# SonyResearch/micro_diffusion

Measured on AMD Instinct MI355X. Metric: training images/sec (global batch 2048) MicroDiT-XL/2 256-res mask=0.75, higher is better.
Workload: dtype bf16; 1 GPU; MicroDiT_XL_2 res_256_pretrain.yaml mask=0.75, full step = 2 microbatches x 1024 fwd+bwd + grad exchange + clip 0.25 + AdamW; global_batch=2048, microbatch=1024, parallelism=dp1, grad_exchange=none (single rank)

## Files before the change

micro_diffusion_amd/csrc/attention.hip:

```cpp
#include <stdlib.h>
#include "md_common.h"
#include "../../include/microdit_hip.h"

namespace {

typedef __attribute__((address_space(3))) s16x4 lds_s16x4;
typedef unsigned int u32x4 __attribute__((ext_vector_type(4)));

__device__ __forceinline__ bf16x4 tr4(const unsigned char* p) {
    s16x4 v = __builtin_amdgcn_ds_read_tr16_b64_v4i16((lds_s16x4*)(p));
    U64 t;
    t.s = v;
    return t.h;
}

__device__ __forceinline__ bf16x8 tr_frag(const unsigned char* tile, int pitch, int k_lo, int k_hi, int col0, int lane) {
    const int li = lane & 15;
    const int col = col0 + ((lane >> 4) & 1) * 16 + (li & 3) * 4;
    const bf16x4 lo = tr4(tile + (k_lo + (li >> 2)) * pitch + col * 2);
    const bf16x4 hi = tr4(tile + (k_hi + (li >> 2)) * pitch + col * 2);
    bf16x8 f;
    f[0] = lo[0]; f[1] = lo[1]; f[2] = lo[2]; f[3] = lo[3];
    f[4] = hi[0]; f[5] = hi[1]; f[6] = hi[2]; f[7] = hi[3];
    return f;
}

__device__ __forceinline__ bf16x8 row_frag(const unsigned char* tile, int pitch, int kbase, int lane) {
    U128 t;
    t.u = *reinterpret_cast<const uint4*>(tile + (lane & 31) * pitch + (kbase + (lane >> 5) * 8) * 2);
    return t.h;
}

template <int HD>
__device__ __forceinline__ void stage_tile(unsigned char* tile, int pitch, const bf16* src, int64_t ld, int64_t row0,
                                           int64_t nrows, int nstage, int tid, int nthreads) {
    constexpr int CPR = HD / 8;
    for (int task = tid; task < nstage * CPR; task += nthreads) {
        const int r = task / CPR, c = task % CPR;
        uint4 v = make_uint4(0, 0, 0, 0);
        if (row0 + r < nrows) v = *reinterpret_cast<const uint4*>(src + (row0 + r) * ld + c * 8);
        *reinterpret_cast<uint4*>(tile + r * pitch + c * 16) = v;
    }
}

constexpr int STG = 32;

template <int HD, int MAXIT>
__device__ __forceinline__ void stage_pair(unsigned char* tileA, unsigned char* tileB, int pitch, const bf16* A, int64_t lda, const bf16* B,
                                           int64_t ldb, int64_t row0, int64_t nrows, int nstage, int tid, int nthreads) {
    constexpr int CPR = HD / 8;
    uint4 ra[MAXIT], rb[MAXIT];
#pragma unroll
    for (int it = 0; it < MAXIT; ++it) {
        const int task = tid + it * nthreads, r = task / CPR, c = task % CPR;
        ra[it] = rb[it] = make_uint4(0, 0, 0, 0);
        if (task < nstage * CPR && row0 + r < nrows) {
            ra[it] = *reinterpret_cast<const uint4*>(A + (row0 + r) * lda + c * 8);
            rb[it] = *reinterpret_cast<const uint4*>(B + (row0 + r) * ldb + c * 8);
        }
    }
#pragma unroll
    for (int it = 0; it < MAXIT; ++it) {
        const int task = tid + it * nthreads, r = task / CPR, c = task % CPR;
        if (task < nstage * CPR) {
            *reinterpret_cast<uint4*>(tileA + r * pitch + c * 16) = ra[it];
            *reinterpret_cast<uint4*>(tileB + r * pitch + c * 16) = rb[it];
        }
    }
}

constexpr float LOG2E = 1.4426950408889634f;
__device__ __forceinline__ int tile_slot(int r, int hh) { return (r & 3) + 8 * (r >> 2) + 4 * hh; }

__device__ __forceinline__ void ds_cols(f32x16& s, const f32x16& dp, float c1, float l2, float dlt, int rem, int hh) {
#pragma unroll
    for (int r = 0; r < 16; ++r) {
        const float pr = tile_slot(r, hh) < rem ? __builtin_amdgcn_exp2f(s[r] * c1 - l2) : 0.f;
        s[r] = pr * (dp[r] - dlt);
    }
}
template <bool WANT_P, bool WANT_DS>
__device__ __forceinline__ void p_ds_rows(f32x16& s, f32x16& dp, float c1, const float* tL2, const float* tDlt, int rem, int hh) {
#pragma unroll
    for (int r = 0; r < 16; ++r) {
        const int ql = tile_slot(r, hh);
        const float pr = ql < rem ? __builtin_amdgcn_exp2f(s[r] * c1 - tL2[ql]) : 0.f;
        if (WANT_DS) dp[r] = pr * (dp[r] - tDlt[ql]);
        if (WANT_P) s[r] = pr;
    }
}
constexpr float LSE_MASKED = 1e30f;
template <bool WANT_P, bool WANT_DS, bool VEC = true>
__device__ __forceinline__ void p_ds_rows_nomask(f32x16& s, f32x16& dp, float c1, const float* tL2, const float* tDlt, int hh) {
    if (!VEC) {
#pragma unroll
        for (int r = 0; r < 16; ++r) {
            const int ql = tile_slot(r, hh);
            const float pr = __builtin_amdgcn_exp2f(s[r] * c1 - tL2[ql]);
            if (WANT_DS) dp[r] = pr * (dp[r] - tDlt[ql]);
            if (WANT_P) s[r] = pr;
        }
        return;
    }
#pragma unroll
    for (int j = 0; j < 4; ++j) {
        const f32x4 l4 = *reinterpret_cast<const f32x4*>(tL2 + 8 * j + 4 * hh);
        f32x4 d4 = {0.f, 0.f, 0.f, 0.f};
        if (WANT_DS) d4 = *reinterpret_cast<const f32x4*>(tDlt + 8 * j + 4 * hh);
#pragma unroll
        for (int e = 0; e < 4; ++e) {
            const int r = 4 * j + e;
            const float pr = __builtin_amdgcn_exp2f(s[r] * c1 - l4[e]);
            if (WANT_DS) dp[r] = pr * (dp[r] - d4[e]);
            if (WANT_P) s[r] = pr;
        }
    }
}

__device__ __forceinline__ bf16x8 pack8(const f32x16& a, int base) {
    bf16x8 o;
#pragma unroll
    for (int e = 0; e < 8; ++e) o[e] = f2bf(a[base + e]);
    return o;
}

__device__ __forceinline__ void bh_of(int64_t lin, int64_t H, int64_t B, int64_t& b, int64_t& h) {
    const int64_t n8 = (B >> 3) * 8 * H;
    if (lin < n8) {
        const int64_t s = lin >> 3, x = lin & 7;
        lin = ((s / H) * 8 + x) * H + s % H;
    }
    b = lin / H;
    h = lin - b * H;
}

enum : unsigned {
    SF_FWD_WIDE = 1u, SF_FWD_LINES = 2u,
    SF_FWDS_WIDE = 4u,
    SF_FUSED_WIDE = 8u, SF_FUSED_LINES = 16u,
    SF_FUSED2_LINES = 32u,
    SF_SPLIT2_WIDE = 64u,
    SF_STREAM_WIDE = 128u, SF_STREAM_LINES = 256u,
// ... 19 lines not shown

template <int HD>
__device__ __forceinline__ void store_rows(bf16* dst_row, const f32x16 (&acc)[HD / 32], float mul, int lane, bool wide) {
    const int hh = lane >> 5;
    if (wide) {
#pragma unroll
        for (int di = 0; di < HD / 32; ++di)
#pragma unroll
            for (int g = 0; g < 4; g += 2) {
                unsigned a0 = cvt_pk_bf16(acc[di][4 * g] * mul, acc[di][4 * g + 1] * mul);
                unsigned a1 = cvt_pk_bf16(acc[di][4 * g + 2] * mul, acc[di][4 * g + 3] * mul);
                unsigned b0 = cvt_pk_bf16(acc[di][4 * g + 4] * mul, acc[di][4 * g + 5] * mul);
                unsigned b1 = cvt_pk_bf16(acc[di][4 * g + 6] * mul, acc[di][4 * g + 7] * mul);
                half_swap(a0, b0);
                half_swap(a1, b1);
                *reinterpret_cast<uint4*>(dst_row + di * 32 + 8 * g + 8 * hh) = make_uint4(a0, a1, b0, b1);
            }
        return;
    }
#pragma unroll
    for (int di = 0; di < HD / 32; ++di)
#pragma unroll
        for (int g = 0; g < 4; ++g) {
            bf16x4 o;
#pragma unroll
            for (int e = 0; e < 4; ++e) o[e] = f2bf(acc[di][4 * g + e] * mul);
            st_bf16x4(dst_row + di * 32 + 8 * g + 4 * hh, o);
        }
}

template <int HD>
__device__ __forceinline__ void store_lines(unsigned char* tile, int pitch, bf16* dst0, int64_t ld, int nvalid, const f32x16 (&acc)[HD / 32],
                                            float mul, int lane) {
    const int hh = lane >> 5;
#pragma unroll
    for (int di = 0; di < HD / 32; ++di)
#pragma unroll
        for (int g = 0; g < 4; ++g)
            *reinterpret_cast<uint2*>(tile + (lane & 31) * pitch + (di * 32 + 8 * g + 4 * hh) * 2) =
                make_uint2(cvt_pk_bf16(acc[di][4 * g] * mul, acc[di][4 * g + 1] * mul), cvt_pk_bf16(acc[di][4 * g + 2] * mul, acc[di][4 * g + 3] * mul));
    __builtin_amdgcn_fence(__ATOMIC_RELEASE, "wavefront");
    __builtin_amdgcn_wave_barrier();
    constexpr int CPR = HD / 8, RPI = 64 / CPR;
#pragma unroll
    for (int it = 0; it < 32 / RPI; ++it) {
        const int r = it * RPI + lane / CPR, c = lane % CPR;
        const uint4 v = *reinterpret_cast<const uint4*>(tile + r * pitch + c * 16);
        if (r < nvalid) *reinterpret_cast<uint4*>(dst0 + r * ld + c * 8) = v;
    }
    __builtin_amdgcn_fence(__ATOMIC_ACQUIRE, "wavefront");
    __builtin_amdgcn_wave_barrier();
}

template <int HD, int MAXIT>
__global__ __launch_bounds__(256) void attn_fwd_kernel(md_attn_args p) {
    constexpr int PK = (HD + 8) * 2;
    __shared__ __attribute__((aligned(16))) unsigned char smem[2 * STG * PK];
    const int tid = threadIdx.x, lane = tid & 63, wave = tid >> 6, nthreads = blockDim.x, nw = nthreads >> 6;
    const int hh = lane >> 5;
    const float c1 = p.scale * LOG2E;
    int64_t b = blockIdx.z, h = blockIdx.y;
    if (gridDim.x == 1) bh_of(blockIdx.y + (int64_t)gridDim.y * blockIdx.z, gridDim.y, gridDim.z, b, h);
    const int64_t q = ((int64_t)blockIdx.x * nw + wave) * 32 + (lane & 31);
    const bool qvalid = q < p.Sq;
    const bf16* Q = reinterpret_cast<const bf16*>(p.q) + b * p.sq + h * p.hsq;
    const bf16* K = reinterpret_cast<const bf16*>(p.k) + b * p.sk + h * p.hsk;
    const bf16* V = reinterpret_cast<const bf16*>(p.v) + b * p.sv + h * p.hsv;

    bf16x8 qf[HD / 16];
#pragma unroll
    for (int s = 0; s < HD / 16; ++s) {
        if (qvalid)
            qf[s] = ld_bf16x8(Q + q * p.ldq + s * 16 + hh * 8);
        else
#pragma unroll
            for (int e = 0; e < 8; ++e) qf[s][e] = f2bf(0.f);
    }
    f32x16 oacc[HD / 32];
#pragma unroll
    for (int di = 0; di < HD / 32; ++di)
#pragma unroll
        for (int r = 0; r < 16; ++r) oacc[di][r] = 0.f;
    float m = -1e30f, l = 0.f;

    for (int64_t kbase = 0; kbase < p.Skv; kbase += STG) {
        __syncthreads();
        const int nst = (int)((p.Skv - kbase >= STG) ? STG : ((p.Skv - kbase + 31) / 32) * 32);
        stage_pair<HD, MAXIT>(smem, smem + STG * PK, PK, K, p.ldk, V, p.ldv, kbase, p.Skv, nst, tid, nthreads);
        __syncthreads();
      for (int sub = 0; sub < STG / 32 && kbase + sub * 32 < p.Skv; ++sub) {
        const int64_t key0 = kbase + sub * 32;
        const unsigned char* sK = smem + sub * 32 * PK;
        const unsigned char* sV = smem + STG * PK + sub * 32 * PK;
        f32x16 sacc;
#pragma unroll
        for (int r = 0; r < 16; ++r) sacc[r] = 0.f;
#pragma unroll
        for (int s = 0; s < HD / 16; ++s)
            sacc = __builtin_amdgcn_mfma_f32_32x32x16_bf16(row_frag(sK, PK, s * 16, lane), qf[s], sacc, 0, 0, 0);
        const int rem = (int)(p.Skv - key0);
        float tmax = -1e30f;
#pragma unroll
        for (int r = 0; r < 16; ++r) {
            sacc[r] = tile_slot(r, hh) < rem ? sacc[r] * c1 : -1e30f;
            tmax = fmaxf(tmax, sacc[r]);
        }
        tmax = fmaxf(tmax, __shfl_xor(tmax, 32, 64));
        const float m_new = fmaxf(m, tmax);
        const float alpha = __builtin_amdgcn_exp2f(m - m_new);
        float psum = 0.f;
#pragma unroll
        for (int r = 0; r < 16; ++r) {
            const float pr = __builtin_amdgcn_exp2f(sacc[r] - m_new);
            sacc[r] = pr;
            psum += pr;
        }
        psum += __shfl_xor(psum, 32, 64);
        l = l * alpha + psum;
        m = m_new;
#pragma unroll
        for (int di = 0; di < HD / 32; ++di)
#pragma unroll
            for (int r = 0; r < 16; ++r) oacc[di][r] *= alpha;
#pragma unroll
        for (int sp = 0; sp < 2; ++sp) {
            const bf16x8 pf = pack8(sacc, 8 * sp);
#pragma unroll
            for (int di = 0; di < HD / 32; ++di)
                oacc[di] = __builtin_amdgcn_mfma_f32_32x32x16_bf16(
                    tr_frag(sV, PK, 16 * sp + 4 * hh, 16 * sp + 8 + 4 * hh, di * 32, lane), pf, oacc[di], 0, 0, 0);
        }
      }
    }
    constexpr bool PLAIN = HD == 64 && MAXIT == 1;
    const bool o16 = rows16(p.o, p.ldo, p.so, p.hso);
    if (sf(SF_FWD_LINES) && !PLAIN && nw <= 2 && o16) {
        __syncthreads();
        const int64_t q0 = ((int64_t)blockIdx.x * nw + wave) * 32;
        const int nvalid = p.Sq - q0 >= 32 ? 32 : (p.Sq > q0 ? (int)(p.Sq - q0) : 0);
        store_lines<HD>(smem + wave * 32 * PK, PK, reinterpret_cast<bf16*>(p.o) + b * p.so + h * p.hso + q0 * p.ldo, p.ldo, nvalid, oacc,
                        1.f / l, lane);
    } else if (qvalid) {
        bf16* O = reinterpret_cast<bf16*>(p.o) + b * p.so + h * p.hso + q * p.ldo;
        store_rows<HD>(O, oacc, 1.f / l, lane, sf(SF_FWD_WIDE) && !PLAIN && o16);
    }
    if (qvalid && lane < 32 && p.lse) reinterpret_cast<float*>(p.lse)[(b * p.H + h) * p.Sq + q] = (m + __log2f(l)) * 0.6931471805599453f;
}


template <int HD, int MAXIT>
struct ChunkRegs {
    u32x4 a[MAXIT], b[MAXIT];
};
template <int HD, int SCH, int MAXIT>
__device__ __forceinline__ void chunk_load(ChunkRegs<HD, MAXIT>& R, const bf16* A, int64_t lda, const bf16* B, int64_t ldb, int64_t row0,
                                           int64_t nrows, int tid, int nthreads) {
    constexpr int CPR = HD / 8;
    const u32x4 z4 = {0u, 0u, 0u, 0u};
#pragma unroll
    for (int it = 0; it < MAXIT; ++it) {
        const int task = tid + it * nthreads, r = task / CPR, c = task % CPR;
        const bool ok = task < SCH * CPR && row0 + r < nrows;
        R.a[it] = ok ? *reinterpret_cast<const u32x4*>(A + (row0 + r) * lda + c * 8) : z4;
        R.b[it] = ok ? *reinterpret_cast<const u32x4*>(B + (row0 + r) * ldb + c * 8) : z4;
    }
}
template <int HD, int SCH, int MAXIT>
__device__ __forceinline__ void chunk_store(const ChunkRegs<HD, MAXIT>& R, unsigned char* tileA, unsigned char* tileB, int pitch, int tid,
                                            int nthreads) {
    constexpr int CPR = HD / 8;
#pragma unroll
    for (int it = 0; it < MAXIT; ++it) {
        const int task = tid + it * nthreads, r = task / CPR, c = task % CPR;
        if (task < SCH * CPR) {
            *reinterpret_cast<u32x4*>(tileA + r * pitch + c * 16) = R.a[it];
            *reinterpret_cast<u32x4*>(tileB + r * pitch + c * 16) = R.b[it];
        }
    }
}

template <int HD, int SCH, int MAXIT>
__global__ __launch_bounds__(512) void attn_fwd_stream_kernel(md_attn_args p) {
    constexpr int PK = (HD + 8) * 2;
    __shared__ __attribute__((aligned(16))) unsigned char smem[2 * SCH * PK];
    unsigned char* sKc = smem;
    unsigned char* sVc = smem + SCH * PK;
    const int tid = threadIdx.x, lane = tid & 63, wave = tid >> 6, nthreads = blockDim.x, nw = nthreads >> 6;
    const int hh = lane >> 5;
    const float c1 = p.scale * LOG2E;
    const int64_t b = blockIdx.z, h = blockIdx.y;
    const int64_t q = ((int64_t)blockIdx.x * nw + wave) * 32 + (lane & 31);
    const bool qvalid = q < p.Sq;
    const bf16* Q = reinterpret_cast<const bf16*>(p.q) + b * p.sq + h * p.hsq;
    const bf16* K = reinterpret_cast<const bf16*>(p.k) + b * p.sk + h * p.hsk;
    const bf16* V = reinterpret_cast<const bf16*>(p.v) + b * p.sv + h * p.hsv;

    ChunkRegs<HD, MAXIT> R;
    chunk_load<HD, SCH, MAXIT>(R, K, p.ldk, V, p.ldv, 0, p.Skv, tid, nthreads);
    bf16x8 qf[HD / 16];
#pragma unroll
    for (int s = 0; s < HD / 16; ++s) {
        if (qvalid)
            qf[s] = ld_bf16x8(Q + q * p.ldq + s * 16 + hh * 8);
        else
#pragma unroll
            for (int e = 0; e < 8; ++e) qf[s][e] = f2bf(0.f);
    }
    f32x16 oacc[HD / 32];
#pragma unroll
    for (int di = 0; di < HD / 32; ++di)
#pragma unroll
        for (int r = 0; r < 16; ++r) oacc[di][r] = 0.f;
    float m = -1e30f, l = 0.f;

    for (int64_t kbase = 0; kbase < p.Skv; kbase += SCH) {
        __syncthreads();
        chunk_store<HD, SCH, MAXIT>(R, sKc, sVc, PK, tid, nthreads);
        __syncthreads();
        if (kbase + SCH < p.Skv) chunk_load<HD, SCH, MAXIT>(R, K, p.ldk, V, p.ldv, kbase + SCH, p.Skv, tid, nthreads);
        auto tile = [&](int sub, int rem) {
            const unsigned char* sK = sKc + sub * 32 * PK;
            const unsigned char* sV = sVc + sub * 32 * PK;
            f32x16 sacc;
#pragma unroll
            for (int r = 0; r < 16; ++r) sacc[r] = 0.f;
#pragma unroll
            for (int s = 0; s < HD / 16; ++s)
                sacc = __builtin_amdgcn_mfma_f32_32x32x16_bf16(row_frag(sK, PK, s * 16, lane), qf[s], sacc, 0, 0, 0);
            float tmax = -1e30f;
#pragma unroll
            for (int r = 0; r < 16; ++r) {
                sacc[r] = tile_slot(r, hh) < rem ? sacc[r] * c1 : -1e30f;
                tmax = fmaxf(tmax, sacc[r]);
            }
            tmax = fmaxf(tmax, __shfl_xor(tmax, 32, 64));
            const float m_new = fmaxf(m, tmax);
            const float alpha = __builtin_amdgcn_exp2f(m - m_new);
            float psum = 0.f;
#pragma unroll
            for (int r = 0; r < 16; ++r) {
                const float pr = __builtin_amdgcn_exp2f(sacc[r] - m_new);
                sacc[r] = pr;
                psum += pr;
            }
            psum += __shfl_xor(psum, 32, 64);
            l = l * alpha + psum;
            m = m_new;
#pragma unroll
            for (int di = 0; di < HD / 32; ++di)
#pragma unroll
                for (int r = 0; r < 16; ++r) oacc[di][r] *= alpha;
#pragma unroll
            for (int sp = 0; sp < 2; ++sp) {
                const bf16x8 pf = pack8(sacc, 8 * sp);
#pragma unroll
                for (int di = 0; di < HD / 32; ++di)
                    oacc[di] = __builtin_amdgcn_mfma_f32_32x32x16_bf16(
                        tr_frag(sV, PK, 16 * sp + 4 * hh, 16 * sp + 8 + 4 * hh, di * 32, lane), pf, oacc[di], 0, 0, 0);
            }
        };
        if (kbase + SCH <= p.Skv) {
#pragma unroll 1
            for (int sub = 0; sub < SCH / 32; ++sub) tile(sub, 32);
        } else {
            for (int sub = 0; sub < SCH / 32 && kbase + sub * 32 < p.Skv; ++sub) tile(sub, (int)(p.Skv - kbase - sub * 32));
        }
    }
    if (qvalid) {
        bf16* O = reinterpret_cast<bf16*>(p.o) + b * p.so + h * p.hso + q * p.ldo;
        store_rows<HD>(O, oacc, 1.f / l, lane, sf(SF_FWDS_WIDE) && rows16(p.o, p.ldo, p.so, p.hso));
        if (lane < 32 && p.lse) reinterpret_cast<float*>(p.lse)[(b * p.H + h) * p.Sq + q] = (m + __log2f(l)) * 0.6931471805599453f;
    }
}

template <int HD, int SCH, int MAXIT>
__global__ __launch_bounds__(512) __attribute__((amdgpu_waves_per_eu((SCH == 64 && MAXIT == 2) ? 3 : 2)))
void attn_bwd_dq_stream_kernel(md_attn_args p) {
    constexpr int PK = (HD + 8) * 2;
    __shared__ __attribute__((aligned(16))) unsigned char smem[2 * SCH * PK];
    unsigned char* sK = smem;
    unsigned char* sV = smem + SCH * PK;
    const int tid = threadIdx.x, lane = tid & 63, wave = tid >> 6, nthreads = blockDim.x, nw = nthreads >> 6;
    const int hh = lane >> 5;
    const int64_t b = blockIdx.z, h = blockIdx.y;
    const int64_t q = ((int64_t)blockIdx.x * nw + wave) * 32 + (lane & 31);
    const bool qvalid = q < p.Sq;
    const bf16* Q = reinterpret_cast<const bf16*>(p.q) + b * p.sq + h * p.hsq;
    const bf16* K = reinterpret_cast<const bf16*>(p.k) + b * p.sk + h * p.hsk;
    const bf16* V = reinterpret_cast<const bf16*>(p.v) + b * p.sv + h * p.hsv;
    const bf16* dO = reinterpret_cast<const bf16*>(p.d_o) + b * p.sdo + h * p.hsdo;

    ChunkRegs<HD, MAXIT> R;
    chunk_load<HD, SCH, MAXIT>(R, K, p.ldk, V, p.ldv, 0, p.Skv, tid, nthreads);
    bf16x8 qf[HD / 16], dof[HD / 16];
#pragma unroll
    for (int s = 0; s < HD / 16; ++s) {
        if (qvalid) {
            qf[s] = ld_bf16x8(Q + q * p.ldq + s * 16 + hh * 8);
            dof[s] = ld_bf16x8(dO + q * p.lddo + s * 16 + hh * 8);
        } else {
#pragma unroll
            for (int e = 0; e < 8; ++e) {
                qf[s][e] = f2bf(0.f);
                dof[s][e] = f2bf(0.f);
// ... 232 lines not shown
            }
            const bf16x8 g = __builtin_bit_cast(bf16x8, rdo[it]), o = __builtin_bit_cast(bf16x8, ro[it]);
            float d = 0.f;
#pragma unroll
            for (int e = 0; e < 8; ++e) d += bf2f(o[e]) * bf2f(g[e]);
#pragma unroll
            for (int s2 = CPR / 2; s2 > 0; s2 >>= 1) d += __shfl_xor(d, s2, 64);
            if (c == 0 && task < SQP * CPR) {
                sDlt[r] = d;
                sLse[r] = rl[it] * LOG2E;
            }
        }
#pragma unroll
        for (int it = 0; it < ITK; ++it) {
            const int task = tid + it * NT, r = task / CPR, c = task % CPR;
            if (task < SKP * CPR) {
                *reinterpret_cast<u32x4*>(sK + r * PK + c * 16) = rk[it];
                *reinterpret_cast<u32x4*>(sV + r * PK + c * 16) = rv[it];
            }
        }
    }
    __syncthreads();

    if (wave < nq32) {
        const unsigned char* myQ = sQ + wave * 32 * PK;
        const unsigned char* mydO = sdO + wave * 32 * PK;
        const int64_t q = (int64_t)wave * 32 + (lane & 31);
        bf16x8 qf[HD / 16], dof[HD / 16];
#pragma unroll
        for (int s = 0; s < HD / 16; ++s) {
            qf[s] = row_frag(myQ, PK, s * 16, lane);
            dof[s] = row_frag(mydO, PK, s * 16, lane);
        }
        const float lse = sLse[wave * 32 + (lane & 31)], dlt = sDlt[wave * 32 + (lane & 31)];
        f32x16 dqacc[HD / 32];
#pragma unroll
        for (int di = 0; di < HD / 32; ++di)
#pragma unroll
            for (int r = 0; r < 16; ++r) dqacc[di][r] = 0.f;
        for (int j = 0; j < nk32; ++j) {
            const unsigned char* tK = sK + j * 32 * PK;
            const unsigned char* tV = sV + j * 32 * PK;
            f32x16 sacc, dpacc;
#pragma unroll
            for (int r = 0; r < 16; ++r) {
                sacc[r] = 0.f;
                dpacc[r] = 0.f;
            }
#pragma unroll
            for (int s = 0; s < HD / 16; ++s) {
                sacc = __builtin_amdgcn_mfma_f32_32x32x16_bf16(row_frag(tK, PK, s * 16, lane), qf[s], sacc, 0, 0, 0);
                dpacc = __builtin_amdgcn_mfma_f32_32x32x16_bf16(row_frag(tV, PK, s * 16, lane), dof[s], dpacc, 0, 0, 0);
            }
            ds_cols(sacc, dpacc, c1, lse, dlt, (int)p.Skv - j * 32, hh);
#pragma unroll
            for (int sp = 0; sp < 2; ++sp) {
                const bf16x8 dsf = pack8(sacc, 8 * sp);
#pragma unroll
                for (int di = 0; di < HD / 32; ++di)
                    dqacc[di] = __builtin_amdgcn_mfma_f32_32x32x16_bf16(
                        tr_frag(tK, PK, 16 * sp + 4 * hh, 16 * sp + 8 + 4 * hh, di * 32, lane), dsf, dqacc[di], 0, 0, 0);
            }
        }
        if (q < p.Sq) {
            bf16* dQ = reinterpret_cast<bf16*>(p.dq) + b * p.sdq + h * p.hsdq + q * p.lddq;
            store_rows<HD>(dQ, dqacc, p.scale, lane, sf(SF_FUSED_WIDE) && rows16(p.dq, p.lddq, p.sdq, p.hsdq));
        }
    }
    f32x16 dkacc[HD / 32], dvacc[HD / 32];
#pragma unroll
    for (int di = 0; di < HD / 32; ++di)
#pragma unroll
        for (int r = 0; r < 16; ++r) {
            dkacc[di][r] = 0.f;
            dvacc[di][r] = 0.f;
        }
    if (wave < nk32) {
        const unsigned char* myK = sK + wave * 32 * PK;
        const unsigned char* myV = sV + wave * 32 * PK;
        bf16x8 kf[HD / 16], vf[HD / 16];
#pragma unroll
        for (int s = 0; s < HD / 16; ++s) {
            kf[s] = row_frag(myK, PK, s * 16, lane);
            vf[s] = row_frag(myV, PK, s * 16, lane);
        }
        for (int i = 0; i < nq32; ++i) {
            const unsigned char* tQ = sQ + i * 32 * PK;
            const unsigned char* tdO = sdO + i * 32 * PK;
            const float* tLse = sLse + i * 32;
            const float* tDlt = sDlt + i * 32;
            f32x16 sacc, dpacc;
#pragma unroll
            for (int r = 0; r < 16; ++r) {
                sacc[r] = 0.f;
                dpacc[r] = 0.f;
            }
#pragma unroll
            for (int s = 0; s < HD / 16; ++s) {
                sacc = __builtin_amdgcn_mfma_f32_32x32x16_bf16(row_frag(tQ, PK, s * 16, lane), kf[s], sacc, 0, 0, 0);
                dpacc = __builtin_amdgcn_mfma_f32_32x32x16_bf16(row_frag(tdO, PK, s * 16, lane), vf[s], dpacc, 0, 0, 0);
            }
            p_ds_rows<true, true>(sacc, dpacc, c1, tLse, tDlt, (int)p.Sq - i * 32, hh);
#pragma unroll
            for (int sp = 0; sp < 2; ++sp) {
                const bf16x8 pf = pack8(sacc, 8 * sp);
                const bf16x8 dsf = pack8(dpacc, 8 * sp);
#pragma unroll
                for (int di = 0; di < HD / 32; ++di) {
                    dvacc[di] = __builtin_amdgcn_mfma_f32_32x32x16_bf16(
                        tr_frag(tdO, PK, 16 * sp + 4 * hh, 16 * sp + 8 + 4 * hh, di * 32, lane), pf, dvacc[di], 0, 0, 0);
                    dkacc[di] = __builtin_amdgcn_mfma_f32_32x32x16_bf16(
                        tr_frag(tQ, PK, 16 * sp + 4 * hh, 16 * sp + 8 + 4 * hh, di * 32, lane), dsf, dkacc[di], 0, 0, 0);
                }
            }
        }
    }
    const bool dk16 = rows16(p.dk, p.lddk, p.sdk, p.hsdk), dv16 = rows16(p.dv, p.lddv, p.sdv, p.hsdv);
    if (sf(SF_FUSED_LINES) && dk16 && dv16) {
        __syncthreads();
        if (wave < nk32) {
            const int nvalid = p.Skv - wave * 32 >= 32 ? 32 : (int)(p.Skv - wave * 32);
            store_lines<HD>(sK + wave * 32 * PK, PK, reinterpret_cast<bf16*>(p.dk) + b * p.sdk + h * p.hsdk + (int64_t)wave * 32 * p.lddk,
                            p.lddk, nvalid, dkacc, p.scale, lane);
            store_lines<HD>(sV + wave * 32 * PK, PK, reinterpret_cast<bf16*>(p.dv) + b * p.sdv + h * p.hsdv + (int64_t)wave * 32 * p.lddv,
                            p.lddv, nvalid, dvacc, 1.f, lane);
        }
    } else if (wave < nk32) {
        const int64_t key = (int64_t)wave * 32 + (lane & 31);
        if (key < p.Skv) {
            bf16* dK = reinterpret_cast<bf16*>(p.dk) + b * p.sdk + h * p.hsdk + key * p.lddk;
            bf16* dV = reinterpret_cast<bf16*>(p.dv) + b * p.sdv + h * p.hsdv + key * p.lddv;
            store_rows<HD>(dK, dkacc, p.scale, lane, sf(SF_FUSED_WIDE) && !sf(SF_FUSED_LINES) && dk16);
            store_rows<HD>(dV, dvacc, 1.f, lane, sf(SF_FUSED_WIDE) && !sf(SF_FUSED_LINES) && dv16);
        }
    }
}

template <int HD, int SQP, int SKP, bool SPLIT2>
__global__ __launch_bounds__((SQP > SKP ? SQP : SKP) * 2) __attribute__((amdgpu_waves_per_eu(SPLIT2 ? 4 : 3)))
void attn_bwd_fused2_kernel(md_attn_args p) {
    constexpr int PK = (HD + 8) * 2;
    constexpr int RMAX = SQP > SKP ? SQP : SKP;
    constexpr int NT = RMAX * 2;
    constexpr bool WIDE = SPLIT2 && sf(SF_SPLIT2_WIDE);
    __shared__ __attribute__((aligned(16))) unsigned char smem[2 * RMAX * PK + 2 * SQP * 4];
    unsigned char* sA = smem;
    unsigned char* sB = smem + RMAX * PK;
    float* sLse = reinterpret_cast<float*>(smem + 2 * RMAX * PK);
    float* sDlt = sLse + SQP;
    const int tid = threadIdx.x, lane = tid & 63, wave = tid >> 6;
    const int hh = lane >> 5;
    const float c1 = p.scale * LOG2E;
    int64_t b, h;
    bh_of(blockIdx.x + (int64_t)gridDim.x * blockIdx.y, gridDim.x, gridDim.y, b, h);
    const bf16* Q = reinterpret_cast<const bf16*>(p.q) + b * p.sq + h * p.hsq;
    const bf16* K = reinterpret_cast<const bf16*>(p.k) + b * p.sk + h * p.hsk;
    const bf16* V = reinterpret_cast<const bf16*>(p.v) + b * p.sv + h * p.hsv;
    const bf16* dO = reinterpret_cast<const bf16*>(p.d_o) + b * p.sdo + h * p.hsdo;
    const bf16* O = reinterpret_cast<const bf16*>(p.o) + b * p.so + h * p.hso;
    const int nq32 = (int)((p.Sq + 31) / 32), nk32 = (int)((p.Skv + 31) / 32);

    constexpr int CPR = HD / 8;
    constexpr int ITQ = (SQP * CPR + NT - 1) / NT, ITK = (SKP * CPR + NT - 1) / NT;
    u32x4 rk[ITK], rv[ITK];
    {
        const float* LSE = reinterpret_cast<const float*>(p.lse) + (b * p.H + h) * p.Sq;
        u32x4 rq[ITQ], rdo[ITQ], ro[ITQ];
        float rl[ITQ];
        const u32x4 z4 = {0u, 0u, 0u, 0u};
#pragma unroll
        for (int it = 0; it < ITQ; ++it) {
            const int task = tid + it * NT, r = task / CPR, c = task % CPR;
            const bool ok = task < SQP * CPR && r < p.Sq;
            rq[it] = ok ? *reinterpret_cast<const u32x4*>(Q + (int64_t)r * p.ldq + c * 8) : z4;
            rdo[it] = ok ? *reinterpret_cast<const u32x4*>(dO + (int64_t)r * p.lddo + c * 8) : z4;
            ro[it] = ok ? *reinterpret_cast<const u32x4*>(O + (int64_t)r * p.ldo + c * 8) : z4;
            rl[it] = (ok && c == 0) ? LSE[r] : 0.f;
        }
#pragma unroll
        for (int it = 0; it < ITK; ++it) {
            const int task = tid + it * NT, r = task / CPR, c = task % CPR;
            const bool ok = task < SKP * CPR && r < p.Skv;
            rk[it] = ok ? *reinterpret_cast<const u32x4*>(K + (int64_t)r * p.ldk + c * 8) : z4;
            rv[it] = ok ? *reinterpret_cast<const u32x4*>(V + (int64_t)r * p.ldv + c * 8) : z4;
        }
#pragma unroll
        for (int it = 0; it < ITQ; ++it) {
            const int task = tid + it * NT, r = task / CPR, c = task % CPR;
            if (task < SQP * CPR) {
                *reinterpret_cast<u32x4*>(sA + r * PK + c * 16) = rq[it];
                *reinterpret_cast<u32x4*>(sB + r * PK + c * 16) = rdo[it];
            }
            const bf16x8 g = __builtin_bit_cast(bf16x8, rdo[it]), o = __builtin_bit_cast(bf16x8, ro[it]);
            float d = 0.f;
#pragma unroll
            for (int e = 0; e < 8; ++e) d += bf2f(o[e]) * bf2f(g[e]);
#pragma unroll
            for (int s2 = CPR / 2; s2 > 0; s2 >>= 1) d += __shfl_xor(d, s2, 64);
            if (c == 0 && task < SQP * CPR) {
                sDlt[r] = d;
                sLse[r] = rl[it] * LOG2E;
            }
        }
    }
    __syncthreads();
    const bool qrole = wave < nq32, krole = wave < nk32;
    bf16x8 qf[HD / 16], dof[HD / 16];
    float lse = 0.f, dlt = 0.f;
    if (qrole) {
#pragma unroll
        for (int s = 0; s < HD / 16; ++s) {
            qf[s] = row_frag(sA + wave * 32 * PK, PK, s * 16, lane);
            dof[s] = row_frag(sB + wave * 32 * PK, PK, s * 16, lane);
        }
        lse = sLse[wave * 32 + (lane & 31)];
        dlt = sDlt[wave * 32 + (lane & 31)];
    }
    __syncthreads();
#pragma unroll
    for (int it = 0; it < ITK; ++it) {
        const int task = tid + it * NT, r = task / CPR, c = task % CPR;
        if (task < SKP * CPR) {
            *reinterpret_cast<u32x4*>(sA + r * PK + c * 16) = rk[it];
            *reinterpret_cast<u32x4*>(sB + r * PK + c * 16) = rv[it];
        }
    }
    __syncthreads();
    if (qrole) {
        const int64_t q = (int64_t)wave * 32 + (lane & 31);
        f32x16 dqacc[HD / 32];
#pragma unroll
        for (int di = 0; di < HD / 32; ++di)
#pragma unroll
            for (int r = 0; r < 16; ++r) dqacc[di][r] = 0.f;
        for (int j = 0; j < nk32; ++j) {
            const unsigned char* tK = sA + j * 32 * PK;
            const unsigned char* tV = sB + j * 32 * PK;
            f32x16 sacc, dpacc;
#pragma unroll
            for (int r = 0; r < 16; ++r) {
                sacc[r] = 0.f;
                dpacc[r] = 0.f;
            }
#pragma unroll
            for (int s = 0; s < HD / 16; ++s) {
                sacc = __builtin_amdgcn_mfma_f32_32x32x16_bf16(row_frag(tK, PK, s * 16, lane), qf[s], sacc, 0, 0, 0);
                dpacc = __builtin_amdgcn_mfma_f32_32x32x16_bf16(row_frag(tV, PK, s * 16, lane), dof[s], dpacc, 0, 0, 0);
            }
            ds_cols(sacc, dpacc, c1, lse, dlt, (int)p.Skv - j * 32, hh);
#pragma unroll
            for (int sp = 0; sp < 2; ++sp) {
                const bf16x8 dsf = pack8(sacc, 8 * sp);
#pragma unroll
                for (int di = 0; di < HD / 32; ++di)
                    dqacc[di] = __builtin_amdgcn_mfma_f32_32x32x16_bf16(
                        tr_frag(tK, PK, 16 * sp + 4 * hh, 16 * sp + 8 + 4 * hh, di * 32, lane), dsf, dqacc[di], 0, 0, 0);
            }
        }
        if (q < p.Sq) {
            bf16* dQ = reinterpret_cast<bf16*>(p.dq) + b * p.sdq + h * p.hsdq + q * p.lddq;
            store_rows<HD>(dQ, dqacc, p.scale, lane, WIDE && rows16(p.dq, p.lddq, p.sdq, p.hsdq));
        }
    }
    bf16x8 kf[HD / 16], vf[HD / 16];
    if (krole) {
#pragma unroll
        for (int s = 0; s < HD / 16; ++s) {
            kf[s] = row_frag(sA + wave * 32 * PK, PK, s * 16, lane);
            vf[s] = row_frag(sB + wave * 32 * PK, PK, s * 16, lane);
        }
    }
    __syncthreads();
    if (qrole) {
#pragma unroll
        for (int s = 0; s < HD / 16; ++s) {
            *reinterpret_cast<u32x4*>(sA + (wave * 32 + (lane & 31)) * PK + (s * 16 + hh * 8) * 2) = __builtin_bit_cast(u32x4, qf[s]);
            *reinterpret_cast<u32x4*>(sB + (wave * 32 + (lane & 31)) * PK + (s * 16 + hh * 8) * 2) = __builtin_bit_cast(u32x4, dof[s]);
        }
    }
    __syncthreads();
    const bool dk16 = rows16(p.dk, p.lddk, p.sdk, p.hsdk), dv16 = rows16(p.dv, p.lddv, p.sdv, p.hsdv);
    const int64_t key = (int64_t)wave * 32 + (lane & 31);
    f32x16 dkacc[HD / 32], dvacc[HD / 32];
#pragma unroll
    for (int di = 0; di < HD / 32; ++di)
#pragma unroll
        for (int r = 0; r < 16; ++r) {
            dkacc[di][r] = 0.f;
            dvacc[di][r] = 0.f;
        }
    if (krole) {
        if (SPLIT2) {
            bf16* dK = reinterpret_cast<bf16*>(p.dk) + b * p.sdk + h * p.hsdk + key * p.lddk;
            bf16* dV = reinterpret_cast<bf16*>(p.dv) + b * p.sdv + h * p.hsdv + key * p.lddv;
            f32x16 acc[HD / 32];
#pragma unroll
            for (int di = 0; di < HD / 32; ++di)
#pragma unroll
                for (int r = 0; r < 16; ++r) acc[di][r] = 0.f;
            for (int i = 0; i < nq32; ++i) {
                const unsigned char* tQ = sA + i * 32 * PK;
                const unsigned char* tdO = sB + i * 32 * PK;
                const float* tLse = sLse + i * 32;
                f32x16 sacc;
#pragma unroll
                for (int r = 0; r < 16; ++r) sacc[r] = 0.f;
#pragma unroll
                for (int s = 0; s < HD / 16; ++s)
                    sacc = __builtin_amdgcn_mfma_f32_32x32x16_bf16(row_frag(tQ, PK, s * 16, lane), kf[s], sacc, 0, 0, 0);
                p_ds_rows<true, false>(sacc, sacc, c1, tLse, nullptr, (int)p.Sq - i * 32, hh);
#pragma unroll
                for (int sp = 0; sp < 2; ++sp) {
                    const bf16x8 pf = pack8(sacc, 8 * sp);
#pragma unroll
                    for (int di = 0; di < HD / 32; ++di)
                        acc[di] = __builtin_amdgcn_mfma_f32_32x32x16_bf16(
                            tr_frag(tdO, PK, 16 * sp + 4 * hh, 16 * sp + 8 + 4 * hh, di * 32, lane), pf, acc[di], 0, 0, 0);
                }
            }
            if (key < p.Skv) {
                store_rows<HD>(dV, acc, 1.f, lane, WIDE && dv16);
            }
#pragma unroll
            for (int di = 0; di < HD / 32; ++di)
#pragma unroll
                for (int r = 0; r < 16; ++r) acc[di][r] = 0.f;
            for (int i = 0; i < nq32; ++i) {
                const unsigned char* tQ = sA + i * 32 * PK;
                const unsigned char* tdO = sB + i * 32 * PK;
                const float* tLse = sLse + i * 32;
                const float* tDlt = sDlt + i * 32;
                f32x16 sacc, dpacc;
#pragma unroll
                for (int r = 0; r < 16; ++r) {
                    sacc[r] = 0.f;
                    dpacc[r] = 0.f;
                }
#pragma unroll
                for (int s = 0; s < HD / 16; ++s) {
                    sacc = __builtin_amdgcn_mfma_f32_32x32x16_bf16(row_frag(tQ, PK, s * 16, lane), kf[s], sacc, 0, 0, 0);
                    dpacc = __builtin_amdgcn_mfma_f32_32x32x16_bf16(row_frag(tdO, PK, s * 16, lane), vf[s], dpacc, 0, 0, 0);
                }
                p_ds_rows<false, true>(sacc, dpacc, c1, tLse, tDlt, (int)p.Sq - i * 32, hh);
#pragma unroll
                for (int sp = 0; sp < 2; ++sp) {
                    const bf16x8 dsf = pack8(dpacc, 8 * sp);
#pragma unroll
                    for (int di = 0; di < HD / 32; ++di)
                        acc[di] = __builtin_amdgcn_mfma_f32_32x32x16_bf16(
                            tr_frag(tQ, PK, 16 * sp + 4 * hh, 16 * sp + 8 + 4 * hh, di * 32, lane), dsf, acc[di], 0, 0, 0);
                }
            }
            if (key < p.Skv) {
                store_rows<HD>(dK, acc, p.scale, lane, WIDE && dk16);
            }
        } else {
            for (int i = 0; i < nq32; ++i) {
                const unsigned char* tQ = sA + i * 32 * PK;
                const unsigned char* tdO = sB + i * 32 * PK;
                const float* tLse = sLse + i * 32;
                const float* tDlt = sDlt + i * 32;
                f32x16 sacc, dpacc;
#pragma unroll
                for (int r = 0; r < 16; ++r) {
                    sacc[r] = 0.f;
                    dpacc[r] = 0.f;
                }
#pragma unroll
                for (int s = 0; s < HD / 16; ++s) {
                    sacc = __builtin_amdgcn_mfma_f32_32x32x16_bf16(row_frag(tQ, PK, s * 16, lane), kf[s], sacc, 0, 0, 0);
                    dpacc = __builtin_amdgcn_mfma_f32_32x32x16_bf16(row_frag(tdO, PK, s * 16, lane), vf[s], dpacc, 0, 0, 0);
                }
                p_ds_rows<true, true>(sacc, dpacc, c1, tLse, tDlt, (int)p.Sq - i * 32, hh);
#pragma unroll
                for (int sp = 0; sp < 2; ++sp) {
                    const bf16x8 pf = pack8(sacc, 8 * sp);
                    const bf16x8 dsf = pack8(dpacc, 8 * sp);
#pragma unroll
                    for (int di = 0; di < HD / 32; ++di) {
                        dvacc[di] = __builtin_amdgcn_mfma_f32_32x32x16_bf16(
                            tr_frag(tdO, PK, 16 * sp + 4 * hh, 16 * sp + 8 + 4 * hh, di * 32, lane), pf, dvacc[di], 0, 0, 0);
                        dkacc[di] = __builtin_amdgcn_mfma_f32_32x32x16_bf16(
                            tr_frag(tQ, PK, 16 * sp + 4 * hh, 16 * sp + 8 + 4 * hh, di * 32, lane), dsf, dkacc[di], 0, 0, 0);
                    }
                }
            }
        }
    }
    if (!SPLIT2) {
        if (sf(SF_FUSED2_LINES) && dk16 && dv16) {
            __syncthreads();
            if (krole) {
                const int nvalid = p.Skv - wave * 32 >= 32 ? 32 : (int)(p.Skv - wave * 32);
                store_lines<HD>(sA + wave * 32 * PK, PK, reinterpret_cast<bf16*>(p.dk) + b * p.sdk + h * p.hsdk + (int64_t)wave * 32 * p.lddk,
                                p.lddk, nvalid, dkacc, p.scale, lane);
                store_lines<HD>(sB + wave * 32 * PK, PK, reinterpret_cast<bf16*>(p.dv) + b * p.sdv + h * p.hsdv + (int64_t)wave * 32 * p.lddv,
                                p.lddv, nvalid, dvacc, 1.f, lane);
            }
        } else if (krole && key < p.Skv) {
            bf16* dK = reinterpret_cast<bf16*>(p.dk) + b * p.sdk + h * p.hsdk + key * p.lddk;
            bf16* dV = reinterpret_cast<bf16*>(p.dv) + b * p.sdv + h * p.hsdv + key * p.lddv;
            store_rows<HD>(dK, dkacc, p.scale, lane, false);
            store_rows<HD>(dV, dvacc, 1.f, lane, false);
        }
    }
}

inline int fused_bucket(int64_t S) { return S <= 64 ? 64 : S <= 96 ? 96 : S <= 256 ? 256 : 0; }

template <int HD>
void launch_bwd_fused_one(const md_attn_args* a, int variant, int bq, int bk, hipStream_t stream) {
    const dim3 grid((unsigned)a->H, (unsigned)a->B);
#define FUSED(SQP, SKP) hipLaunchKernelGGL((attn_bwd_fused_kernel<HD, SQP, SKP>), grid, dim3((SQP > SKP ? SQP : SKP) * 2), 0, stream, *a)
#define FUSED2(SQP, SKP, SPL) \
    hipLaunchKernelGGL((attn_bwd_fused2_kernel<HD, SQP, SKP, SPL>), grid, dim3((SQP > SKP ? SQP : SKP) * 2), 0, stream, *a)
#define SMALL(SQP, SKP)                          \
    do {                                         \
        if (variant == 2 || (variant == 0 && SQP == 64 && SKP == 64)) FUSED(SQP, SKP); \
        else if (variant == 4) FUSED2(SQP, SKP, true); \
        else FUSED2(SQP, SKP, false);            \
    } while (0)
#define BIG(SQP, SKP)                            \
    do {                                         \
        if (variant == 2) FUSED(SQP, SKP);       \
        else FUSED2(SQP, SKP, true);             \
    } while (0)
// ... 132 lines not shown
```

micro_diffusion_amd/hip.py:

```python
from __future__ import annotations

import ctypes
import os
from ctypes import c_float, c_int, c_int32, c_int64, c_void_p, POINTER, Structure, byref

from . import native

_CSRC = native.CSRC
_HEADER = os.path.join(native.INCLUDE, "microdit_hip.h")
LIB_PATH = os.path.join(os.path.dirname(_CSRC), "libmicrodit_hip.so")

HIPCC_FLAGS = ["--offload-arch=gfx950", "-O3", "-std=c++17", "-fPIC", "-munsafe-fp-atomics",
               "-Wno-unused-result", "-Wno-inline-asm"]

ACT_NONE, ACT_GELU_TANH, ACT_GELU_ERF, ACT_SILU = 0, 1, 2, 3
EPI_STORE_BF16, EPI_RESIDUAL, EPI_STORE_F32, EPI_ACCUM_F32, EPI_ATOMIC_F32, EPI_DACT, EPI_SWIGLU_BWD = 0, 1, 2, 3, 4, 5, 6
DET_GATE_BWD, DET_LN_BWD, DET_COLSUM = 0, 1, 2
GEMM_AUTO, GEMM_REG128, GEMM_DMA128, GEMM_PACED256, GEMM_PP256, GEMM_W4 = 0, 1, 2, 3, 4, 5
GEMM_VARIANT_NAMES = {"auto": 0, "reg128": 1, "dma128": 2, "paced256": 3, "pp256": 4, "w4": 5}
ATTN_BWD_AUTO, ATTN_BWD_FUSED_1PHASE, ATTN_BWD_FUSED_2PHASE, ATTN_BWD_FUSED_2PHASE_SPLIT, ATTN_BWD_STREAM_PAIR = 0, 2, 3, 4, 5


def _hashed_files():
    return [os.path.join(_CSRC, f) for f in sorted(os.listdir(_CSRC)) if os.path.isfile(os.path.join(_CSRC, f))] + [_HEADER]


def _gemm_source_hash() -> str:
    files = [os.path.join(_CSRC, f) for f in sorted(os.listdir(_CSRC))
             if f.endswith((".hip", ".h", ".inc")) and (f.startswith("gemm") or f == "md_common.h")]
    return native.source_hash(files + [_HEADER], HIPCC_FLAGS)


def _source_hash() -> str:
    return native.source_hash(_hashed_files(), HIPCC_FLAGS)


def build(force: bool = False, verbose: bool = True) -> str:
    def make(tmp):
        hipcc = native.hipcc()
        objdir = os.path.join(_CSRC, "build")
        os.makedirs(objdir, exist_ok=True)
        srcs = sorted(f for f in os.listdir(_CSRC) if f.endswith(".hip"))
        objs = [os.path.join(objdir, f[:-4] + ".o") for f in srcs]
        native.run(*([hipcc, *HIPCC_FLAGS, "-I", native.INCLUDE, "-c", os.path.join(_CSRC, f), "-o", o] for f, o in zip(srcs, objs)),
                   verbose=verbose)
        native.run([hipcc, "--offload-arch=gfx950", "-shared", "-fPIC", *objs, "-o", tmp])
    return native.build(LIB_PATH, _source_hash(), make, force)


class GemmProblem(Structure):
    _fields_ = [("A", c_void_p), ("B", c_void_p), ("lda", c_int64), ("ldb", c_int64), ("M", c_int64), ("N", c_int64), ("c_off", c_int64)]


GEMM_MAX_PROBLEMS = 8
NUM_CU = 256


class GemmArgs(Structure):
    _fields_ = [
        ("A", c_void_p), ("B", c_void_p), ("C", c_void_p), ("C2", c_void_p), ("bias", c_void_p),
        ("res", c_void_p), ("gate", c_void_p), ("aux", c_void_p),
        ("M", c_int64), ("N", c_int64), ("K", c_int64),
        ("lda", c_int64), ("ldb", c_int64), ("ldc", c_int64), ("ldc2", c_int64), ("ldr", c_int64),
        ("ldg", c_int64), ("ldaux", c_int64),
        ("sA", c_int64), ("sB", c_int64), ("sC", c_int64), ("sC2", c_int64), ("sBias", c_int64),
        ("sAux", c_int64), ("sSplit", c_int64),
        ("rows_per_sample", c_int64),
        ("batch", c_int32), ("ksplit", c_int32), ("a_kcontig", c_int32), ("b_kcontig", c_int32),
        ("mode", c_int32), ("act", c_int32), ("alpha", c_float), ("variant", c_int32), ("raster_group_n", c_int32),
        ("timeline", c_void_p), ("chosen_variant", c_void_p), ("A_list", c_void_p), ("B_list", c_void_p), ("list_segments", c_int32),
        ("problems", c_void_p), ("n_problems", c_int32), ("cu_limit", c_int32),
        ("tail_ws", c_void_p), ("tail_ws_bytes", c_int64), ("tail_mode", c_int32), ("tail_used", c_void_p),
        ("dact_cached", c_int32),
    ]


_lib = None
ABI_VERSION = 6


def lib() -> ctypes.CDLL:
    global _lib
    if _lib is None:
        path = os.environ.get("MICRODIT_LIB")
        if not path:
            stale = not native.up_to_date(LIB_PATH, _source_hash())
            if stale and (os.path.exists("/opt/rocm/bin/hipcc") or os.environ.get("HIPCC")):
                build()
            if not os.path.exists(LIB_PATH):
                raise RuntimeError(
                    f"{LIB_PATH} is missing: the MicroDiT HIP extension has not been built. "
                    "Run `python -c 'import __graft_entry__ as g; g.build()'` (needs hipcc). "
                    "There is no CPU / PyTorch fallback for the training path.")
            path = LIB_PATH
        _lib = native.load(path, _SIGS, "md_abi_version", ABI_VERSION)
    return _lib


NOT_ELIGIBLE = -2

# ... 265 lines not shown
```

Baseline: 2907 images/sec.

## Add packed-VALU, mask-free whole-tile, and rescale-skip softmax forms to attention kernels

Adds compile-time variants of the attention softmax and dS/P elementwise code. They use packed f32x2 math for exp and FMA, skip per-element masking when a 32-key tile is full, and skip the output rescale when no row max increased, checked with a wave ballot. The forward kernel also gets a waves-per-EU attribute. Defaults enable most forms for head dim 64, aiming to cut VALU work in the attention inner loops. The risks are register pressure or occupancy changes and small numeric differences from the changed rounding and contraction.

Measured after the change: 2931 images/sec, median of 6. About the same (+0.8%).

```diff
diff --git a/micro_diffusion_amd/csrc/attention.hip b/micro_diffusion_amd/csrc/attention.hip
--- a/micro_diffusion_amd/csrc/attention.hip
+++ b/micro_diffusion_amd/csrc/attention.hip
@@ -72,22 +72,86 @@
 constexpr float LOG2E = 1.4426950408889634f;
 __device__ __forceinline__ int tile_slot(int r, int hh) { return (r & 3) + 8 * (r >> 2) + 4 * hh; }
 
+enum : unsigned {
+    VF_FWD_WHOLE = 1u, VF_FWD_PK = 2u, VF_FWD_SKIP = 4u, VF_FWD_VACC = 8u,
+    VF_FWDS_SKIP = 16u,
+    VF_FUSED_WHOLE = 32u, VF_FUSED_PK = 64u,
+    VF_SPLIT2_PK = 128u,
+};
+#ifndef MD_ATTN_VALU_FORMS
+#define MD_ATTN_VALU_FORMS 0xedu
+#endif
+constexpr bool vform(unsigned bit) { return (MD_ATTN_VALU_FORMS & bit) != 0; }
+#if (MD_ATTN_VALU_FORMS) & 8u
+#define MD_ATTN_FWD_WAVES __attribute__((amdgpu_waves_per_eu(HD == 64 ? 2 : 1)))
+#else
+#define MD_ATTN_FWD_WAVES
+#endif
+
+__device__ __forceinline__ f32x2 exp2_2(f32x2 x) { return f32x2{__builtin_amdgcn_exp2f(x.x), __builtin_amdgcn_exp2f(x.y)}; }
+
+template <bool MASK, bool PK>
+__device__ __forceinline__ void ds_cols_body(f32x16& s, const f32x16& dp, float c1, float l2, float dlt, int rem, int hh) {
+    if (PK) {
+#pragma unroll
+        for (int r = 0; r < 16; r += 2) {
+            f32x2 pr = exp2_2(__builtin_elementwise_fma(f32x2{s[r], s[r + 1]}, f32x2{c1, c1}, f32x2{-l2, -l2}));
+            if (MASK) {
+                pr.x = tile_slot(r, hh) < rem ? pr.x : 0.f;
+                pr.y = tile_slot(r + 1, hh) < rem ? pr.y : 0.f;
+            }
+            const f32x2 d = pr * (f32x2{dp[r], dp[r + 1]} - dlt);
+            s[r] = d.x;
+            s[r + 1] = d.y;
+        }
+        return;
+    }
+#pragma unroll
+    for (int r = 0; r < 16; ++r) {
+        const float pr = (!MASK || tile_slot(r, hh) < rem) ? __builtin_amdgcn_exp2f(s[r] * c1 - l2) : 0.f;
+        s[r] = pr * (dp[r] - dlt);
+    }
+}
+template <bool WHOLE = false, bool PK = false>
 __device__ __forceinline__ void ds_cols(f32x16& s, const f32x16& dp, float c1, float l2, float dlt, int rem, int hh) {
-#pragma unroll
-    for (int r = 0; r < 16; ++r) {
-        const float pr = tile_slot(r, hh) < rem ? __builtin_amdgcn_exp2f(s[r] * c1 - l2) : 0.f;
-        s[r] = pr * (dp[r] - dlt);
-    }
-}
-template <bool WANT_P, bool WANT_DS>
-__device__ __forceinline__ void p_ds_rows(f32x16& s, f32x16& dp, float c1, const float* tL2, const float* tDlt, int rem, int hh) {
+    if (WHOLE && rem >= 32) ds_cols_body<false, PK>(s, dp, c1, l2, dlt, rem, hh);
+    else ds_cols_body<true, PK>(s, dp, c1, l2, dlt, rem, hh);
+}
+template <bool WANT_P, bool WANT_DS, bool MASK, bool PK>
+__device__ __forceinline__ void p_ds_rows_body(f32x16& s, f32x16& dp, float c1, const float* tL2, const float* tDlt, int rem, int hh) {
+    if (PK) {
+#pragma unroll
+        for (int r = 0; r < 16; r += 2) {
+            const int ql = tile_slot(r, hh);
+            f32x2 pr = exp2_2(__builtin_elementwise_fma(f32x2{s[r], s[r + 1]}, f32x2{c1, c1}, f32x2{-tL2[ql], -tL2[ql + 1]}));
+            if (MASK) {
+                pr.x = ql < rem ? pr.x : 0.f;
+                pr.y = ql + 1 < rem ? pr.y : 0.f;
+            }
+            if (WANT_DS) {
+                const f32x2 d = pr * (f32x2{dp[r], dp[r + 1]} - f32x2{tDlt[ql], tDlt[ql + 1]});
+                dp[r] = d.x;
+                dp[r + 1] = d.y;
+            }
+            if (WANT_P) {
+                s[r] = pr.x;
+                s[r + 1] = pr.y;
+            }
+        }
+        return;
+    }
 #pragma unroll
     for (int r = 0; r < 16; ++r) {
         const int ql = tile_slot(r, hh);
-        const float pr = ql < rem ? __builtin_amdgcn_exp2f(s[r] * c1 - tL2[ql]) : 0.f;
+        const float pr = (!MASK || ql < rem) ? __builtin_amdgcn_exp2f(s[r] * c1 - tL2[ql]) : 0.f;
         if (WANT_DS) dp[r] = pr * (dp[r] - tDlt[ql]);
         if (WANT_P) s[r] = pr;
     }
+}
+template <bool WANT_P, bool WANT_DS, bool WHOLE = false, bool PK = false>
+__device__ __forceinline__ void p_ds_rows(f32x16& s, f32x16& dp, float c1, const float* tL2, const float* tDlt, int rem, int hh) {
+    if (WHOLE && rem >= 32) p_ds_rows_body<WANT_P, WANT_DS, false, PK>(s, dp, c1, tL2, tDlt, rem, hh);
+    else p_ds_rows_body<WANT_P, WANT_DS, true, PK>(s, dp, c1, tL2, tDlt, rem, hh);
 }
 constexpr float LSE_MASKED = 1e30f;
 template <bool WANT_P, bool WANT_DS, bool VEC = true>
@@ -213,9 +277,94 @@
     __builtin_amdgcn_wave_barrier();
 }
 
+__device__ __forceinline__ float mul_rn(float a, float b) {
+#pragma clang fp contract(off)
+    return a * b;
+}
+__device__ __forceinline__ f32x2 mul_rn(f32x2 a, float b) {
+#pragma clang fp contract(off)
+    return a * b;
+}
+template <bool MASK, bool PK>
+__device__ __forceinline__ float scale_max(f32x16& sacc, float c1, int rem, int hh) {
+    float tmax = -1e30f;
+    if (PK) {
+#pragma unroll
+        for (int r = 0; r < 16; r += 2) {
+            f32x2 t = mul_rn(f32x2{sacc[r], sacc[r + 1]}, c1);
+            if (MASK) {
+                t.x = tile_slot(r, hh) < rem ? t.x : -1e30f;
+                t.y = tile_slot(r + 1, hh) < rem ? t.y : -1e30f;
+            }
+            sacc[r] = t.x;
+            sacc[r + 1] = t.y;
+            tmax = fmaxf(fmaxf(tmax, t.x), t.y);
+        }
+    } else {
+#pragma unroll
+        for (int r = 0; r < 16; ++r) {
+            if (MASK) sacc[r] = tile_slot(r, hh) < rem ? sacc[r] * c1 : -1e30f;
+            else sacc[r] = mul_rn(sacc[r], c1);
+            tmax = fmaxf(tmax, sacc[r]);
+        }
+    }
+    return tmax;
+}
+template <int HD, bool WHOLE, bool PK, bool SKIP>
+__device__ __forceinline__ void softmax_step(f32x16& sacc, f32x16 (&oacc)[HD / 32], float& m, float& l, float c1, int rem, int hh) {
+    float tmax;
+    if (WHOLE && rem >= 32) tmax = scale_max<false, PK>(sacc, c1, rem, hh);
+    else tmax = scale_max<true, PK>(sacc, c1, rem, hh);
+    tmax = fmaxf(tmax, __shfl_xor(tmax, 32, 64));
+    const float m_new = fmaxf(m, tmax);
+    float psum = 0.f;
+    if (PK) {
+#pragma unroll
+        for (int r = 0; r < 16; r += 2) {
+            const f32x2 pr = exp2_2(f32x2{sacc[r], sacc[r + 1]} - m_new);
+            sacc[r] = pr.x;
+            sacc[r + 1] = pr.y;
+            psum += pr.x;
+            psum += pr.y;
+        }
+    } else {
+#pragma unroll
+        for (int r = 0; r < 16; ++r) {
+            const float pr = __builtin_amdgcn_exp2f(sacc[r] - m_new);
+            sacc[r] = pr;
+            psum += pr;
+        }
+    }
+    psum += __shfl_xor(psum, 32, 64);
+    if (SKIP && __builtin_amdgcn_ballot_w64(tmax > m) == 0) {
+        l += psum;
+        return;
+    }
+    const float alpha = __builtin_amdgcn_exp2f(m - m_new);
+    l = __builtin_fmaf(l, alpha, psum);
+    m = m_new;
+    if (PK) {
+#pragma unroll
+        for (int di = 0; di < HD / 32; ++di)
+#pragma unroll
+            for (int r = 0; r < 16; r += 2) {
+                const f32x2 o = f32x2{oacc[di][r], oacc[di][r + 1]} * alpha;
+                oacc[di][r] = o.x;
+                oacc[di][r + 1] = o.y;
+            }
+    } else {
+#pragma unroll
+        for (int di = 0; di < HD / 32; ++di)
+#pragma unroll
+            for (int r = 0; r < 16; ++r) oacc[di][r] *= alpha;
+    }
+}
+
 template <int HD, int MAXIT>
-__global__ __launch_bounds__(256) void attn_fwd_kernel(md_attn_args p) {
+__global__ __launch_bounds__(256) MD_ATTN_FWD_WAVES void attn_fwd_kernel(md_attn_args p) {
     constexpr int PK = (HD + 8) * 2;
+    constexpr bool FWHOLE = HD == 64 && vform(VF_FWD_WHOLE), FSKIP = HD == 64 && vform(VF_FWD_SKIP);
+    constexpr bool FPK = HD == 64 && vform(VF_FWD_PK) && !(MAXIT == 1 && FWHOLE && FSKIP);
     __shared__ __attribute__((aligned(16))) unsigned char smem[2 * STG * PK];
     const int tid = threadIdx.x, lane = tid & 63, wave = tid >> 6, nthreads = blockDim.x, nw = nthreads >> 6;
     const int hh = lane >> 5;
@@ -260,29 +409,7 @@
         for (int s = 0; s < HD / 16; ++s)
             sacc = __builtin_amdgcn_mfma_f32_32x32x16_bf16(row_frag(sK, PK, s * 16, lane), qf[s], sacc, 0, 0, 0);
         const int rem = (int)(p.Skv - key0);
-        float tmax = -1e30f;
-#pragma unroll
-        for (int r = 0; r < 16; ++r) {
-            sacc[r] = tile_slot(r, hh) < rem ? sacc[r] * c1 : -1e30f;
-            tmax = fmaxf(tmax, sacc[r]);
-        }
-        tmax = fmaxf(tmax, __shfl_xor(tmax, 32, 64));
-        const float m_new = fmaxf(m, tmax);
-        const float alpha = __builtin_amdgcn_exp2f(m - m_new);
-        float psum = 0.f;
-#pragma unroll
-        for (int r = 0; r < 16; ++r) {
-            const float pr = __builtin_amdgcn_exp2f(sacc[r] - m_new);
-            sacc[r] = pr;
-            psum += pr;
-        }
-        psum += __shfl_xor(psum, 32, 64);
-        l = l * alpha + psum;
-        m = m_new;
-#pragma unroll
-        for (int di = 0; di < HD / 32; ++di)
-#pragma unroll
-            for (int r = 0; r < 16; ++r) oacc[di][r] *= alpha;
+        softmax_step<HD, FWHOLE, FPK, FSKIP>(sacc, oacc, m, l, c1, rem, hh);
 #pragma unroll
         for (int sp = 0; sp < 2; ++sp) {
             const bf16x8 pf = pack8(sacc, 8 * sp);
@@ -388,29 +515,7 @@
 #pragma unroll
             for (int s = 0; s < HD / 16; ++s)
                 sacc = __builtin_amdgcn_mfma_f32_32x32x16_bf16(row_frag(sK, PK, s * 16, lane), qf[s], sacc, 0, 0, 0);
-            float tmax = -1e30f;
-#pragma unroll
-            for (int r = 0; r < 16; ++r) {
-                sacc[r] = tile_slot(r, hh) < rem ? sacc[r] * c1 : -1e30f;
-                tmax = fmaxf(tmax, sacc[r]);
-            }
-            tmax = fmaxf(tmax, __shfl_xor(tmax, 32, 64));
-            const float m_new = fmaxf(m, tmax);
-            const float alpha = __builtin_amdgcn_exp2f(m - m_new);
-            float psum = 0.f;
-#pragma unroll
-            for (int r = 0; r < 16; ++r) {
-                const float pr = __builtin_amdgcn_exp2f(sacc[r] - m_new);
-                sacc[r] = pr;
-                psum += pr;
-            }
-            psum += __shfl_xor(psum, 32, 64);
-            l = l * alpha + psum;
-            m = m_new;
-#pragma unroll
-            for (int di = 0; di < HD / 32; ++di)
-#pragma unroll
-                for (int r = 0; r < 16; ++r) oacc[di][r] *= alpha;
+            softmax_step<HD, false, false, HD == 64 && vform(VF_FWDS_SKIP)>(sacc, oacc, m, l, c1, rem, hh);
 #pragma unroll
             for (int sp = 0; sp < 2; ++sp) {
                 const bf16x8 pf = pack8(sacc, 8 * sp);
@@ -749,7 +854,7 @@
                 sacc = __builtin_amdgcn_mfma_f32_32x32x16_bf16(row_frag(tK, PK, s * 16, lane), qf[s], sacc, 0, 0, 0);
                 dpacc = __builtin_amdgcn_mfma_f32_32x32x16_bf16(row_frag(tV, PK, s * 16, lane), dof[s], dpacc, 0, 0, 0);
             }
-            ds_cols(sacc, dpacc, c1, lse, dlt, (int)p.Skv - j * 32, hh);
+            ds_cols<HD == 64 && vform(VF_FUSED_WHOLE), HD == 64 && vform(VF_FUSED_PK)>(sacc, dpacc, c1, lse, dlt, (int)p.Skv - j * 32, hh);
 #pragma unroll
             for (int sp = 0; sp < 2; ++sp) {
                 const bf16x8 dsf = pack8(sacc, 8 * sp);
@@ -797,7 +902,7 @@
                 sacc = __builtin_amdgcn_mfma_f32_32x32x16_bf16(row_frag(tQ, PK, s * 16, lane), kf[s], sacc, 0, 0, 0);
                 dpacc = __builtin_amdgcn_mfma_f32_32x32x16_bf16(row_frag(tdO, PK, s * 16, lane), vf[s], dpacc, 0, 0, 0);
             }
-            p_ds_rows<true, true>(sacc, dpacc, c1, tLse, tDlt, (int)p.Sq - i * 32, hh);
+            p_ds_rows<true, true, HD == 64 && vform(VF_FUSED_WHOLE), HD == 64 && vform(VF_FUSED_PK)>(sacc, dpacc, c1, tLse, tDlt, (int)p.Sq - i * 32, hh);
 #pragma unroll
             for (int sp = 0; sp < 2; ++sp) {
                 const bf16x8 pf = pack8(sacc, 8 * sp);
@@ -840,6 +945,7 @@
     constexpr int RMAX = SQP > SKP ? SQP : SKP;
     constexpr int NT = RMAX * 2;
     constexpr bool WIDE = SPLIT2 && sf(SF_SPLIT2_WIDE);
+    constexpr bool VPK = HD == 64 && SPLIT2 && vform(VF_SPLIT2_PK);
     __shared__ __attribute__((aligned(16))) unsigned char smem[2 * RMAX * PK + 2 * SQP * 4];
     unsigned char* sA = smem;
     unsigned char* sB = smem + RMAX * PK;
@@ -944,7 +1050,7 @@
                 sacc = __builtin_amdgcn_mfma_f32_32x32x16_bf16(row_frag(tK, PK, s * 16, lane), qf[s], sacc, 0, 0, 0);
                 dpacc = __builtin_amdgcn_mfma_f32_32x32x16_bf16(row_frag(tV, PK, s * 16, lane), dof[s], dpacc, 0, 0, 0);
             }
-            ds_cols(sacc, dpacc, c1, lse, dlt, (int)p.Skv - j * 32, hh);
+            ds_cols<false, VPK>(sacc, dpacc, c1, lse, dlt, (int)p.Skv - j * 32, hh);
 #pragma unroll
             for (int sp = 0; sp < 2; ++sp) {
                 const bf16x8 dsf = pack8(sacc, 8 * sp);
@@ -1005,7 +1111,7 @@
 #pragma unroll
                 for (int s = 0; s < HD / 16; ++s)
                     sacc = __builtin_amdgcn_mfma_f32_32x32x16_bf16(row_frag(tQ, PK, s * 16, lane), kf[s], sacc, 0, 0, 0);
-                p_ds_rows<true, false>(sacc, sacc, c1, tLse, nullptr, (int)p.Sq - i * 32, hh);
+                p_ds_rows<true, false, false, VPK>(sacc, sacc, c1, tLse, nullptr, (int)p.Sq - i * 32, hh);
 #pragma unroll
                 for (int sp = 0; sp < 2; ++sp) {
                     const bf16x8 pf = pack8(sacc, 8 * sp);
@@ -1038,7 +1144,7 @@
                     sacc = __builtin_amdgcn_mfma_f32_32x32x16_bf16(row_frag(tQ, PK, s * 16, lane), kf[s], sacc, 0, 0, 0);
                     dpacc = __builtin_amdgcn_mfma_f32_32x32x16_bf16(row_frag(tdO, PK, s * 16, lane), vf[s], dpacc, 0, 0, 0);
                 }
-                p_ds_rows<false, true>(sacc, dpacc, c1, tLse, tDlt, (int)p.Sq - i * 32, hh);
+                p_ds_rows<false, true, false, VPK>(sacc, dpacc, c1, tLse, tDlt, (int)p.Sq - i * 32, hh);
 #pragma unroll
                 for (int sp = 0; sp < 2; ++sp) {
                     const bf16x8 dsf = pack8(dpacc, 8 * sp);
@@ -1068,7 +1174,7 @@
                     sacc = __builtin_amdgcn_mfma_f32_32x32x16_bf16(row_frag(tQ, PK, s * 16, lane), kf[s], sacc, 0, 0, 0);
                     dpacc = __builtin_amdgcn_mfma_f32_32x32x16_bf16(row_frag(tdO, PK, s * 16, lane), vf[s], dpacc, 0, 0, 0);
                 }
-                p_ds_rows<true, true>(sacc, dpacc, c1, tLse, tDlt, (int)p.Sq - i * 32, hh);
+                p_ds_rows<true, true, false, VPK>(sacc, dpacc, c1, tLse, tDlt, (int)p.Sq - i * 32, hh);
 #pragma unroll
                 for (int sp = 0; sp < 2; ++sp) {
                     const bf16x8 pf = pack8(sacc, 8 * sp);
diff --git a/micro_diffusion_amd/hip.py b/micro_diffusion_amd/hip.py
--- a/micro_diffusion_amd/hip.py
+++ b/micro_diffusion_amd/hip.py
@@ -46,6 +46,11 @@
                    verbose=verbose)
         native.run([hipcc, "--offload-arch=gfx950", "-shared", "-fPIC", *objs, "-o", tmp])
     return native.build(LIB_PATH, _source_hash(), make, force)
+
+
+def build_side_library(src: str, out: str, *defines: str) -> str:
+    native.run([native.hipcc(), *HIPCC_FLAGS, *defines, "-I", native.INCLUDE, "-shared", os.path.join(_CSRC, src), "-o", str(out)])
+    return str(out)
 
 
 class GemmProblem(Structure):
```
